# CN-UPB/DeepCoMP

Hardware: AMD Instinct MI355X
Metric: env steps/sec (higher is better)
Workload: dtype f64 positions / f32 rates

## Files before the change

deepcomp_amd/csrc/dcomp_device.h:

```cpp
#pragma once
#include <hip/hip_runtime.h>
#include <stdint.h>

#include "../../include/dcomp_types.h"

#define DCOMP_BLOCK 256
#define DCOMP_WIDE_MIN_B 20
#define DCOMP_SPARSE_MIN_B 7

#define VM_ARRIVED1(a) asm volatile("" : "+v"(a))
#define VM_ARRIVED2(a, b) asm volatile("" : "+v"(a), "+v"(b))
#define VM_ARRIVED3(a, b, c) asm volatile("" : "+v"(a), "+v"(b), "+v"(c))

namespace dcomp {

constexpr float BW = 9e6f;
constexpr float LOG2E = 1.4426950408889634f;
constexpr float TEN_LOG10_2 = 3.0102999566398120f;
constexpr float EPS = 1e-16f;
constexpr float MIN_UTIL = -20.f, MAX_UTIL = 20.f;

struct UeCfg {
    int16_t init_x, init_y;
    uint8_t vel_lo, vel_hi;
// ... 45 lines not shown
    uint32_t maxcap_mask;
    double pl_c1, pl_c2;
    uint32_t time;
    int32_t num_steps;
    int32_t out_every_step;
    int32_t horizon;
    int32_t tight_g;
    int32_t tight_gpw;
    int32_t tight_magic;
    uint32_t episode_inc;
    uint32_t any_sum_mode;
    uint32_t seed_lo, seed_hi, episode;
    uint32_t env_base;
    float half_gamma;
    float log2k;
    float log2k_s;
    double dt2;
    float dt2f;
    uint32_t dsq_exact;
    double bs_x[DCOMP_MASK32_MAX_BS], bs_y[DCOMP_MASK32_MAX_BS];
    int32_t bs_mode[DCOMP_MASK32_MAX_BS];
};

template <int CTRL>
__device__ __forceinline__ float dpp_f32(float v)
{
    return __int_as_float(__builtin_amdgcn_update_dpp(0, __float_as_int(v), CTRL, 0xF, 0xF, true));
}
__device__ __forceinline__ float swz_xor16(float v)
{
    return __int_as_float(__builtin_amdgcn_ds_swizzle(__float_as_int(v), 0x401F));
}
#define DCOMP_DPP_QUAD_X1 0xB1
#define DCOMP_DPP_QUAD_X2 0x4E
#define DCOMP_DPP_HALF_MIRROR 0x141
#define DCOMP_DPP_ROW_MIRROR 0x140

struct OpSum { __device__ __forceinline__ static float f(float a, float b) { return a + b; } };
struct OpMin { __device__ __forceinline__ static float f(float a, float b) { return __builtin_amdgcn_fmed3f(a, b, -3.0e38f); } };
struct OpMax { __device__ __forceinline__ static float f(float a, float b) { return __builtin_amdgcn_fmed3f(a, b, 3.0e38f); } };

template <int W, class Op>
__device__ __forceinline__ float group_reduce(float v)
{
    if (W >= 2) v = Op::f(v, dpp_f32<DCOMP_DPP_QUAD_X1>(v));
    if (W >= 4) v = Op::f(v, dpp_f32<DCOMP_DPP_QUAD_X2>(v));
// ... 107 lines not shown
    return xx + yy;
}
__device__ __noinline__ bool in_range_exact(double px, double py, double bx, double by, double dt2)
{
    return dist_sq_ref(bx - px, by - py) < dt2;
}
__device__ __forceinline__ void pair_eval_q(double px, double py, double bx, double by, const KParams &p, bool &in_range, float &l2snr, float &q);
__device__ __forceinline__ void pair_eval(double px, double py, double bx, double by, const KParams &p, bool &in_range,
                                          float &l2snr, bool &tiny)
{
    float q;
    pair_eval_q(px, py, bx, by, p, in_range, l2snr, q);
    tiny = q < NEAR_D2;
    if (q == p.dt2f || p.dsq_exact) in_range = in_range_exact(px, py, bx, by, p.dt2);
}
__device__ __forceinline__ void pair_eval_q(double px, double py, double bx, double by, const KParams &p, bool &in_range, float &l2snr, float &q)
{
    double dx = bx - px, dy = by - py;
    double dsq = __builtin_fma(dy, dy, dx * dx);
    in_range = dsq < p.dt2;
    q = (float)dsq;
    l2snr = __builtin_fmaf(-p.half_gamma, fast_log2(q * 0x1p-12f), p.log2k_s);
}
__device__ __forceinline__ float pair_eval_tiny(double px, double py, double bx, double by, const KParams &p)
{
    double dx = bx - px, dy = by - py;
    float q = (float)__builtin_fma(dy, dy, dx * dx);
    float d = __builtin_amdgcn_sqrtf(q) + EPS;
    return __builtin_fmaf(-2.0f * p.half_gamma, fast_log2(d), p.log2k);
}
template <int B>
__device__ __forceinline__ uint32_t eval_pairs(double px, double py, const KParams &p, float (&l2)[B], bool *near_wave = nullptr,
                                               const double *bsx = nullptr, const double *bsy = nullptr)
{
    uint32_t in_range = 0;
    float qmin = 3.0e38f;
    const bool vec_form = bsx != nullptr;
    bool edge = false;
    float emin = 3.0e38f;
#pragma unroll
    for (int b = 0; b < B; b++) {
        bool ir;
        float q;
        pair_eval_q(px, py, bsx ? bsx[b] : p.bs_x[b], bsy ? bsy[b] : p.bs_y[b], p, ir, l2[b], q);
        in_range |= (uint32_t)ir << b;
        qmin = min_med3(qmin, q);
        if (vec_form) emin = min_med3(emin, __builtin_fabsf(q - p.dt2f));
        else edge |= q == p.dt2f;
    }
    if (vec_form) edge = emin == 0.f;
    if (__ballot(edge) != 0ull || p.dsq_exact) {
        in_range = 0;
#pragma unroll
        for (int b = 0; b < B; b++)
            in_range |= (uint32_t)in_range_exact(px, py, bsx ? bsx[b] : p.bs_x[b], bsy ? bsy[b] : p.bs_y[b], p.dt2) << b;
    }
    const bool nw = __ballot(qmin < NEAR_D2) != 0ull;
    if (near_wave) *near_wave = nw;
    if (nw) {
#pragma unroll
        for (int b = 0; b < B; b++) {
            const double bx = bsx ? bsx[b] : p.bs_x[b], by = bsy ? bsy[b] : p.bs_y[b];
            float t = pair_eval_tiny(px, py, bx, by, p);
            double dx = bx - px, dy = by - py;
            if ((float)__builtin_fma(dy, dy, dx * dx) < 1e-20f) l2[b] = t;
        }
    }
    return in_range;
}
constexpr float RATE_SMALL_L2 = -6.0f + L2_OFF;
__device__ __forceinline__ float rate_unshared_small(float l2snr, bool &needfix)
{
    needfix = l2snr > RATE_SMALL_L2;
    const float z = fast_exp2(min_med3(l2snr, RATE_SMALL_L2));
    constexpr float K = BW * LOG2E, S1 = 0x1p-24f, S2 = 0x1p-48f, S3 = 0x1p-72f, S4 = 0x1p-96f;
    float t = __builtin_fmaf(z, -0.25f * K * S4, 0.33333334f * K * S3);
    t = __builtin_fmaf(z, t, -0.5f * K * S2);
    t = __builtin_fmaf(z, t, K * S1);
    return z * t;
}
__device__ __forceinline__ float rate_unshared_any(float l2snr)
{
    const float l = l2snr - L2_OFF;
    const float s = fast_exp2(fminf(l, 100.f));
    const float u = 1.0f + s;
    const float lg = fast_log2(u) * (s * fast_rcp(u - 1.0f));
// ... 8 lines not shown
}

__device__ __forceinline__ void philox4x32_10(uint32_t c0, uint32_t c1, uint32_t c2, uint32_t c3, uint32_t k0, uint32_t k1,
                                              uint32_t (&out)[4])
{
#pragma unroll
    for (int r = 0; r < 10; r++) {
        const unsigned long long p0 = (unsigned long long)0xD2511F53u * c0, p1 = (unsigned long long)0xCD9E8D57u * c2;
        const uint32_t hi0 = (uint32_t)(p0 >> 32), lo0 = (uint32_t)p0, hi1 = (uint32_t)(p1 >> 32), lo1 = (uint32_t)p1;
        c0 = hi1 ^ c1 ^ k0; c1 = lo1; c2 = hi0 ^ c3 ^ k1; c3 = lo0;
        k0 += 0x9E3779B9u; k1 += 0xBB67AE85u;
    }
    out[0] = c0; out[1] = c1; out[2] = c2; out[3] = c3;
}

__device__ __forceinline__ unsigned long long mv_pack(uint32_t wx, uint32_t wy, uint32_t vel, uint32_t pausing, uint32_t cp,
                                                      uint32_t cursor)
{
    return (unsigned long long)(wx & 0xFFFF) | ((unsigned long long)(wy & 0xFFFF) << 16) | ((unsigned long long)(vel & 0xFF) << 32) |
           ((unsigned long long)((pausing << 7) | (cp & 0x7Fu)) << 40) | ((unsigned long long)(cursor & 0xFFFF) << 48);
}

constexpr uint32_t UID_BORN = 0x8000u;
__device__ __forceinline__ void draw_triple(const KParams &p, int env, uint32_t uidw, uint32_t k, uint32_t episode, uint32_t &vel,
                                            uint32_t &wx, uint32_t &wy, int mcfg)
{
    const uint32_t id0 = (uidw & 0x7FFFu) - 1u;
    const bool born = (uidw & UID_BORN) != 0u;
    if (p.rng_mode == DCOMP_RNG_TAPE) {
        if (k >= (uint32_t)p.tape_depth) { atomicOr(p.flags, DCOMP_FLAG_TAPE_EMPTY); k = p.tape_depth - 1; }
        const uint32_t slot = born ? (uint32_t)p.U0 + id0 : id0;
        ushort4 t = p.tape_triples[((size_t)env * p.tape_ids + slot) * p.tape_depth + k];
        vel = t.x; wx = t.y; wy = t.z;
        VM_ARRIVED3(vel, wx, wy);
    } else {
        uint32_t r[4] = {0x12345678u + k * 977u, 0x9abcdef0u ^ uidw * 2654435761u, 0x0fedcba9u + (uint32_t)env * 40503u, 0u};
        philox4x32_10(p.env_base + (uint32_t)env, id0 | (born ? UID_BORN : 0u), episode, k + 1, p.seed_lo, p.seed_hi, r);
        const uint32_t vlo = (uint32_t)mcfg & 0xFFu, vhi = ((uint32_t)mcfg >> 8) & 0xFFu, bb = ((uint32_t)mcfg >> 23) & 0xFFu;
        vel = vlo + __umulhi(r[0], vhi - vlo + 1u);
        wx = bb + __umulhi(r[1], (uint32_t)(p.map_w - 2 * (int)bb + 1));
        wy = bb + __umulhi(r[2], (uint32_t)(p.map_h - 2 * (int)bb + 1));
    }
}
template <bool SCALAR>
__device__ __forceinline__ void draw_triple_wave(const KParams &p, int env, uint32_t uidw, uint32_t k, uint32_t episode, bool redraw,
                                                 uint32_t &vel, uint32_t &wx, uint32_t &wy, int mcfg)
{
    if (!SCALAR || p.rng_mode == DCOMP_RNG_TAPE) {
        if (redraw) draw_triple(p, env, uidw, k, episode, vel, wx, wy, mcfg);
        return;
    }
    const int lane = (int)(threadIdx.x & 63u);
    unsigned long long need = __ballot(redraw);
    while (need != 0ull) {
        const int l = __ffsll((long long)need) - 1;
        need &= need - 1ull;
        uint32_t k0 = p.seed_lo, k1 = p.seed_hi, eb = p.env_base;
        asm volatile("" : "+s"(k0), "+s"(k1), "+s"(eb));
        const uint32_t e_s = (uint32_t)__builtin_amdgcn_readlane(env, l), u_s = (uint32_t)__builtin_amdgcn_readlane((int)uidw, l);
        const uint32_t k_s = (uint32_t)__builtin_amdgcn_readlane((int)k, l), m_s = (uint32_t)__builtin_amdgcn_readlane(mcfg, l);
        uint32_t r[4] = {0x12345678u + k_s * 977u, 0x9abcdef0u ^ u_s * 2654435761u, 0x0fedcba9u + e_s * 40503u, 0u};
        philox4x32_10(eb + e_s, ((u_s & 0x7FFFu) - 1u) | (u_s & UID_BORN), episode, k_s + 1u, k0, k1, r);
        const uint32_t vlo = m_s & 0xFFu, vhi = (m_s >> 8) & 0xFFu, bb = (m_s >> 23) & 0xFFu;
        const uint32_t v_s = vlo + __umulhi(r[0], vhi - vlo + 1u);
        const uint32_t x_s = bb + __umulhi(r[1], (uint32_t)(p.map_w - 2 * (int)bb + 1));
        const uint32_t y_s = bb + __umulhi(r[2], (uint32_t)(p.map_h - 2 * (int)bb + 1));
        const bool mine = lane == l;
        vel = mine ? v_s : vel; wx = mine ? x_s : wx; wy = mine ? y_s : wy;
    }
}
__device__ __forceinline__ int load_mv_cfg(const KParams &p, uint32_t uidw)
{
// ... 67 lines not shown
        }
    }
}

template <bool LAT = false>
__device__ __forceinline__ void move_ue(const KParams &p, int env, uint32_t uidw, uint32_t episode, double &px, double &py,
                                        unsigned long long &mv, int mcfg)
{
#pragma clang fp contract(off)
    uint32_t wxi = (uint32_t)(mv & 0xFFFF), wyi = (uint32_t)((mv >> 16) & 0xFFFF), vel = (uint32_t)((mv >> 32) & 0xFF);
    uint32_t pz = (uint32_t)((mv >> 40) & 0xFF), cursor = (uint32_t)(mv >> 48);
    uint32_t pausing = (pz >> 7) & 1, cp = pz & 0x7Fu;
    const uint32_t pause_dur = ((uint32_t)mcfg >> 16) & 0x7Fu;
    double wx = (double)wxi, wy = (double)wyi;
    if (px == wx && py == wy) pausing = 1;
    const bool stay = pausing && cp < pause_dur;
    const bool redraw = pausing && !stay;
    cp = stay ? cp + 1u : cp;
    draw_triple_wave<LAT>(p, env, uidw, cursor, episode, redraw, vel, wxi, wyi, mcfg);
    cursor = redraw ? cursor + 1u : cursor;
    pausing = redraw ? 0u : pausing;
    cp = redraw ? 0u : cp;
    wx = (double)wxi; wy = (double)wyi;
    if (p.ue_velq != nullptr) advance_ue<LAT, true>(p, uidw, vel, stay, wx, wy, px, py);
    else advance_ue<LAT, false>(p, uidw, vel, stay, wx, wy, px, py);
    mv = mv_pack(wxi, wyi, vel, pausing, cp, cursor);
}

enum { MP_GENERIC = 0, MP_RES_FAIR = 1, MP_MIXED = 2 };
template <int MP>
__device__ __forceinline__ int bs_mode_of(const KParams &p, int b)
{
    if (MP == MP_RES_FAIR) return DCOMP_RES_FAIR;
    if (MP == MP_MIXED) return (b % 3 == 0) ? DCOMP_RES_FAIR : (b % 3 == 1) ? DCOMP_RATE_FAIR : DCOMP_PROP_FAIR;
    return p.bs_mode[b];
}

template <int B, int UPAD>
struct Geo {
    static constexpr int WG = UPAD < 64 ? UPAD : 64;
    static constexpr int NW = UPAD > 64 ? UPAD / 64 : 1;
    static constexpr int GPB = DCOMP_BLOCK >= UPAD ? DCOMP_BLOCK / UPAD : 1;
    static constexpr int ROW_MULTI = 4 * B + 1;
};

template <int B>
struct StageGeo {
// ... 42 lines not shown
        v[i] = a;
    }
    __syncthreads();
}

__device__ __noinline__ unsigned long long maxcap_rate_key(double pl_c1, double pl_c2, double px, double py, double bx, double by)
{
#pragma clang fp contract(off)
    const double dx = bx - px, dy = by - py;
    const double d = __builtin_sqrt(dx * dx + dy * dy);
    const double pl = pl_c1 + pl_c2 * log10(d + 1e-16);
    const double snr = pow(10.0, (30.0 - pl) / 10.0) / 1e-9;
    return (unsigned long long)__double_as_longlong(1.0 + snr);
}

template <int B, int UPAD, int MP, class S = SegPadded, bool PRE = false, int CARRY = 0>
__device__ __forceinline__ void shared_rates(const KParams &p, BlockSharedT<B, UPAD> &sh, uint32_t conn, const float (&l2)[B], float ewma,
                                             double px, double py, int u, int idx, int env_local, int wave, int lane, int gbase,
                                             float (&dr)[B], float (&cnt)[B], int near_hint = -1, const S &sg = S{}, const float *prow = nullptr,
                                             float *dru_io = nullptr)
{
    using G = Geo<B, UPAD>;
    float agg[B];
    const float inv_ewma = fast_rcp(ewma + EPS);
    bool fix = false;
#pragma unroll
    for (int b = 0; b < B; b++) {
        const bool c = (conn >> b) & 1u;
        unsigned long long m = __ballot(c);
        float dru = 0.f;
        if (PRE) dru = c ? prow[b] : 0.f;
        else if (CARRY == 2) dru = c ? dru_io[b] : 0.f;
        else if (CARRY == 1) {
            bool f;
            const float t = rate_unshared_small(l2[b], f);
            dru_io[b] = t;
            dru = c ? t : 0.f;
        } else if (m != 0ull) {
            bool f;
            const float t = rate_unshared_small(l2[b], f);
            dru = c ? t : 0.f;
            if (near_hint < 0) fix |= c && f;
        }
        dr[b] = dru;
        cnt[b] = (float)seg_popcount<G::WG>(m, gbase, sg);
    }
    if (!PRE && CARRY != 2 && (near_hint < 0 ? (__ballot(fix) != 0ull) : (near_hint != 0))) {
#pragma unroll
        for (int b = 0; b < B; b++) {
            if (CARRY == 1) { if (l2[b] > RATE_SMALL_L2) { dru_io[b] = rate_unshared_any(l2[b]); if ((conn >> b) & 1u) dr[b] = dru_io[b]; } }
            else if (((conn >> b) & 1u) && l2[b] > RATE_SMALL_L2) dr[b] = rate_unshared_any(l2[b]);
        }
    }
#pragma unroll
    for (int b = 0; b < B; b++) {
        const bool c = (conn >> b) & 1u;
        const int mode = bs_mode_of<MP>(p, b);
        float a = 0.f;
        if (mode == DCOMP_RATE_FAIR) a = c ? fast_rcp(dr[b]) : 0.f;
        else if (mode == DCOMP_PROP_FAIR) a = dr[b] * inv_ewma;
        agg[b] = a;
    }
    if (MP == MP_MIXED) {
        constexpr int NS = B - (B + 2) / 3;
        if (NS > 0) {
            float sv[NS > 0 ? NS : 1];
#pragma unroll
            for (int b = 0, k = 0; b < B; b++) if (b % 3 != 0) sv[k++] = agg[b];
// ... 38 lines not shown
#pragma unroll
        for (int b = 0; b < B; b++) {
            key[b] = 1ull;
            if (heavy && ((contested >> b) & 1u)) key[b] = maxcap_rate_key(p.pl_c1, p.pl_c2, px, py, p.bs_x[b], p.bs_y[b]);
            if ((cand >> b) & 1u) atomicMax(&sh.mc_u[env_local * B + b], key[b]);
        }
        __syncthreads();
#pragma unroll
        for (int b = 0; b < B; b++)
            if (((cand >> b) & 1u) && key[b] == sh.mc_u[env_local * B + b])
                atomicMin(&sh.mc_win[env_local * B + b], ((uint32_t)p.conn_since[(size_t)idx * B + b] << 8) | (uint32_t)u);
        __syncthreads();
#pragma unroll
        for (int b = 0; b < B; b++)
            if (((cand >> b) & 1u) && (sh.mc_win[env_local * B + b] & 0xFFu) == (uint32_t)u) mc_winner |= 1u << b;
        __syncthreads();
    }
#pragma unroll
    for (int b = 0; b < B; b++) {
#pragma clang fp contract(off)
        const bool c = (conn >> b) & 1u;
        const int mode = bs_mode_of<MP>(p, b);
        float dru = dr[b], out = 0.f;
        if (mode == DCOMP_RES_FAIR) out = dru * fast_rcp(fmaxf(cnt[b], 1.f));
        else if (mode == DCOMP_RATE_FAIR) out = fast_rcp(agg[b]);
        else if (mode == DCOMP_PROP_FAIR) out = (dru * inv_ewma) * fast_rcp(agg[b] + EPS) * dru;
        else out = ((mc_winner >> b) & 1u) ? dru : 0.f;
        dr[b] = (mode == DCOMP_RES_FAIR || mode == DCOMP_PROP_FAIR) ? out : (c ? out : 0.f);
    }
}

struct Outs { float *obs, *reward, *sum_util, *ue_dr, *ue_util, *rb_out; uint8_t *next_act; int compact; };

template <int B, class F>
__device__ __forceinline__ int policy_action_fn(const KParams &p, uint32_t conn, F dr)
{
    float mx = dr(0);
    int best = 0;
#pragma unroll 4
    for (int b = 1; b < B; b++) { const float d = dr(b); if (d > mx) { mx = d; best = b; } }
    if (p.policy == DCOMP_POLICY_3GPP) return ((conn >> best) & 1u) ? 0 : conn ? __builtin_ffs((int)conn) : best + 1;
    uint32_t sel = B == 32 ? ~0u : (1u << (B & 31)) - 1u;
    if (p.policy == DCOMP_POLICY_DYNAMIC) {
        const float thr = mx * p.policy_eps;
        sel = 0;
#pragma unroll 4
        for (int b = 0; b < B; b++) sel |= (dr(b) >= thr ? 1u : 0u) << b;
    } else if (p.policy == DCOMP_POLICY_CLUSTER) { sel = p.policy_cluster[best]; VM_ARRIVED1(sel); }
    const uint32_t drop = conn & ~sel;
    if (drop) return __builtin_ffs((int)drop);
    const uint32_t cand = sel & ~conn;
    float m2 = -__builtin_huge_valf();
    int a = 0;
#pragma unroll 4
    for (int b = 0; b < B; b++) { const float d = dr(b); if (((cand >> b) & 1u) && d > m2) { m2 = d; a = b + 1; } }
// ... 5 lines not shown
{
    float mx = dr[0];
    int best = 0;
#pragma unroll
    for (int b = 1; b < B; b++) if (dr[b] > mx) { mx = dr[b]; best = b; }
    if (p.policy == DCOMP_POLICY_3GPP)
        return ((conn >> best) & 1u) ? 0 : conn ? __builtin_ffs((int)conn) : best + 1;
    uint32_t sel = B == 32 ? ~0u : (1u << (B & 31)) - 1u;
    if (p.policy == DCOMP_POLICY_DYNAMIC) {
        const float thr = mx * p.policy_eps;
        sel = 0;
#pragma unroll
        for (int b = 0; b < B; b++) sel |= (dr[b] >= thr ? 1u : 0u) << b;
    } else if (p.policy == DCOMP_POLICY_CLUSTER) { sel = p.policy_cluster[best]; VM_ARRIVED1(sel); }
    const uint32_t drop = conn & ~sel;
    if (drop) return __builtin_ffs((int)drop);
    const uint32_t cand = sel & ~conn;
    float m2 = -__builtin_huge_valf();
    int a = 0;
#pragma unroll
    for (int b = 0; b < B; b++) if (((cand >> b) & 1u) && dr[b] > m2) { m2 = dr[b]; a = b + 1; }
    return a;
}
template <int B, int UPAD, bool RESET, bool DYN = false, bool STAGED = true, class S = SegPadded, int POL = -1, int KIND = -1>
__device__ __forceinline__ void write_outputs(const KParams &p, const Outs &o, BlockSharedT<B, UPAD> &sh, bool active, int env, int env_local, int u, int idx,
                                              int wave, int lane, int gbase, uint32_t conn, uint32_t in_range,
                                              float (&l2)[B], float (&cnt)[B], float util, float curr_dr,
                                              float reward_before, bool alive, int n_eff, const S &sg = S{}, uint32_t *pol_next = nullptr)
{
    using G = Geo<B, UPAD>;
    using SG = StageGeo<B>;
    const int U = p.U;
    const int kind = KIND >= 0 ? KIND : p.kind;
    float tsum[B];
#pragma unroll
    for (int b = 0; b < B; b++) tsum[b] = ((conn >> b) & 1u) ? util : 0.f;
    if (!RESET && kind == DCOMP_MULTI) {
        seg_reduce_vec<G::WG, OpSum, B>(tsum, sg, lane);
        if (G::NW > 1) xwave_reduce_<B, G::NW, OpSum>(tsum, sh, wave, lane);
    }
    float l2max = l2[0];
#pragma unroll
    for (int b = 1; b < B; b++) l2max = fmaxf(l2max, l2[b]);

    float reward = 0.f;
    if (kind == DCOMP_CENTRAL) {
        float r[1];
        if (p.reward_agg == DCOMP_REWARD_MIN) {
            r[0] = seg_reduce<G::WG, OpMin>(alive ? reward_before : 1.f, sg, lane);
            xwave_reduce_<1, G::NW, OpMin>(r, sh, wave, lane);
        } else {
            r[0] = seg_reduce<G::WG, OpSum>(alive ? reward_before : 0.f, sg, lane);
            xwave_reduce_<1, G::NW, OpSum>(r, sh, wave, lane);
            if (p.reward_agg == DCOMP_REWARD_AVG) r[0] = r[0] * fast_rcp((float)n_eff);
        }
        reward = r[0];
    } else if (!RESET) {
        reward = util;
        if (p.reward_agg == DCOMP_REWARD_SUM) {
            sh.nb_conn[threadIdx.x] = alive ? conn : 0u;
            sh.nb_rb[threadIdx.x] = reward_before;
            __syncthreads();
            if (in_range != 0) {
                float s = 0.f;
                const int base = (int)threadIdx.x - u;
                for (int v = 0; v < U; v++) if (sh.nb_conn[base + v] & conn) s += sh.nb_rb[base + v];
                reward = s;
            }
            __syncthreads();
        } else {
            if (p.reward_agg == DCOMP_REWARD_AVG) {
                float n = 0.f, t = 0.f;
#pragma unroll
                for (int b = 0; b < B; b++) {
                    const float ind = (float)((in_range >> b) & 1u);
                    n = __builtin_fmaf(ind, cnt[b], n);
                    t = __builtin_fmaf(ind, tsum[b], t);
                }
                if (n > 0.f) {
                    const bool lone = conn == 0u;
                    reward = (lone ? t + util : t) * fast_rcp(lone ? n + 1.f : n);
                }
            } else {
                float tmin[B];
#pragma unroll
                for (int b = 0; b < B; b++) tmin[b] = ((conn >> b) & 1u) ? util : MAX_UTIL;
                seg_reduce_vec<G::WG, OpMin, B>(tmin, sg, lane);
                if (G::NW > 1) xwave_reduce_<B, G::NW, OpMin>(tmin, sh, wave, lane);
                float m = util;
#pragma unroll
                for (int b = 0; b < B; b++) if ((in_range >> b) & 1u) m = fminf(m, cnt[b] > 0.f ? tmin[b] : MAX_UTIL);
                reward = (in_range != 0) ? m : util;
            }
        }
    }

    if (o.sum_util) {
        float s[1];
        s[0] = seg_reduce<G::WG, OpSum>(alive ? util : 0.f, sg, lane);
        xwave_reduce_<1, G::NW, OpSum>(s, sh, wave, lane);
        if (active && u == 0) o.sum_util[env] = s[0];
    }
    if (active) {
        if (o.ue_dr) stream_store(&o.ue_dr[idx], alive ? curr_dr : 0.f);
        if (o.ue_util) stream_store(&o.ue_util[idx], alive ? util : 0.f);
        if (o.rb_out) stream_store(&o.rb_out[idx], alive ? reward_before : 0.f);
    }

    const float inv_u = fast_rcp((float)n_eff);
    const bool live = DYN ? alive : true;
    const float util_n = live ? util * (1.0f / MAX_UTIL) : 0.f;
    float env_cols[DYN ? 2 * B : 1];
#pragma unroll
    for (int b = 0; b < B; b++) {
        l2[b] = live ? fast_exp2(l2[b] - l2max) : 0.f;
        const float avg = tsum[b] * fast_rcp(fmaxf(cnt[b], 1.f)) * (1.0f / MAX_UTIL);
        if (DYN) { env_cols[b] = cnt[b] * inv_u; env_cols[B + b] = avg; }
        tsum[b] = live ? avg : 0.f;
        cnt[b] = live ? cnt[b] * inv_u : 0.f;
    }
    if (POL != 0 && (POL == 1 || o.next_act)) {
        const int a = policy_action<B>(p, conn, l2);
        if (active && o.next_act) o.next_act[idx] = (uint8_t)(live ? a : 0);
        if (pol_next) *pol_next = live ? (uint32_t)a : 0u;
    }
    if (kind == DCOMP_MULTI && !STAGED) {
        if (active && o.compact) {
            if (o.reward) o.reward[idx] = alive ? reward : 0.f;
            float *rec = o.obs + (size_t)idx * (B + 2) + (size_t)env * (2 * B);
            float recv[B + 2];
#pragma unroll
            for (int b = 0; b < B; b++) recv[b] = l2[b];
            recv[B] = util_n;
            recv[B + 1] = __uint_as_float(conn);
            store_run<B + 2>(rec, recv);
            if (u == U - 1) {
                float tl[2 * B];
#pragma unroll
                for (int b = 0; b < B; b++) { tl[b] = cnt[b]; tl[B + b] = tsum[b]; }
                store_run<2 * B>(rec + B + 2, tl);
            }
        } else if (active) {
            if (o.reward) o.reward[idx] = alive ? reward : 0.f;
            float rowv[SG::ROW];
#pragma unroll
            for (int b = 0; b < B; b++) {
                rowv[b] = (float)((conn >> b) & 1u);
                rowv[B + b] = l2[b];
                rowv[2 * B + b] = cnt[b];
                rowv[3 * B + b] = tsum[b];
            }
            rowv[4 * B] = util_n;
            store_run<SG::ROW>(o.obs + (size_t)idx * SG::ROW, rowv);
        }
    } else if (kind == DCOMP_MULTI && o.compact) {
        if (active && o.reward) stream_store(&o.reward[idx], alive ? reward : 0.f);
        const unsigned long long am = __ballot(active);
        if (am != 0ull) {
            constexpr int CW = B + 2;
            const int first = __ffsll((long long)am) - 1, last = 63 - __clzll((long long)am);
            const int idx0 = __builtin_amdgcn_readlane(idx, first), env0 = __builtin_amdgcn_readlane(env, first);
            const size_t g0 = (size_t)idx0 * CW + (size_t)env0 * (2 * B);
            const int loc = (idx - idx0) * CW + (env - env0) * (2 * B);
            const bool tail = u == U - 1;
            const int n = __builtin_amdgcn_readlane(loc + CW + (tail ? 2 * B : 0), last);
            const int ph = (int)((((size_t)o.obs >> 2) + g0) & 3);
            uint32_t *st = reinterpret_cast<uint32_t *>(sh.stage[wave]);
            constexpr int CH = (SG::WORDS - 4) & ~3;
            const bool one = n <= CH;
#pragma unroll 1
            for (int w0 = 0; w0 < n; w0 += CH) {
                const int cw = min(CH, n - w0);
                if (active) {
                    uint32_t *rec = st + ph - w0 + loc;
                    const int at = loc - w0;
#pragma unroll
                    for (int b = 0; b < B; b++) if (one || (unsigned)(at + b) < (unsigned)cw) rec[b] = __float_as_uint(l2[b]);
                    if (one || (unsigned)(at + B) < (unsigned)cw) rec[B] = __float_as_uint(util_n);
                    if (one || (unsigned)(at + B + 1) < (unsigned)cw) rec[B + 1] = conn;
                    if (tail) {
#pragma unroll
                        for (int b = 0; b < B; b++) {
                            if (one || (unsigned)(at + CW + b) < (unsigned)cw) rec[CW + b] = __float_as_uint(DYN ? env_cols[b] : cnt[b]);
                            if (one || (unsigned)(at + CW + B + b) < (unsigned)cw) rec[CW + B + b] = __float_as_uint(DYN ? env_cols[B + b] : tsum[b]);
                        }
                    }
                }
                wave_lds_fence();
                const int n_end = ph + cw;
                uint32_t *gbase_ptr = reinterpret_cast<uint32_t *>(o.obs) + g0 + w0 - ph;
                for (int j = lane * 4; j < n_end; j += 256) {
                    if (j >= ph && j + 4 <= n_end) {
                        typedef uint32_t u4v __attribute__((ext_vector_type(4)));
                        __builtin_nontemporal_store(*reinterpret_cast<const u4v *>(st + j), reinterpret_cast<u4v *>(gbase_ptr + j));
                    } else {
                        for (int k = max(j, ph); k < min(j + 4, n_end); k++) gbase_ptr[k] = st[k];
                    }
                }
                wave_lds_fence();
            }
        }
    } else if (kind == DCOMP_MULTI) {
        if (active && o.reward) stream_store(&o.reward[idx], alive ? reward : 0.f);
        const unsigned long long am = __ballot(active);
        const int nrows = group_popcount<64>(am, 0);
        const int row0 = __builtin_amdgcn_readlane(idx, am ? __ffsll((long long)am) - 1 : 0);
        const int r = idx - row0;
        float *st = sh.stage[wave];
#pragma unroll 1
        for (int pass = 0; pass < SG::NPASS; pass++) {
            const int rbase = pass * SG::RPP;
            if (rbase >= nrows) break;
            const int rows = min(SG::RPP, nrows - rbase);
            const size_t g0 = (size_t)(row0 + rbase) * SG::ROW;
            const int ph = (int)((((size_t)o.obs >> 2) + g0) & 3);
            if (active && r >= rbase && r < rbase + rows) {
                float *row = st + ph + (r - rbase) * SG::ROW;
#pragma unroll
                for (int b = 0; b < B; b++) {
                    row[b] = (float)((conn >> b) & 1u);
                    row[B + b] = l2[b];
                    row[2 * B + b] = cnt[b];
                    row[3 * B + b] = tsum[b];
                }
                row[4 * B] = util_n;
            }
            wave_lds_fence();
            const int n_end = ph + rows * SG::ROW;
            float *gbase_ptr = o.obs + g0 - ph;
            for (int j = lane * 4; j < n_end; j += 256) {
                if (j >= ph && j + 4 <= n_end) {
                    typedef float f4v __attribute__((ext_vector_type(4)));
                    __builtin_nontemporal_store(*reinterpret_cast<const f4v *>(st + j), reinterpret_cast<f4v *>(gbase_ptr + j));
                } else {
                    for (int k = max(j, ph); k < min(j + 4, n_end); k++) gbase_ptr[k] = st[k];
                }
            }
            wave_lds_fence();
        }
    } else if (G::NW == 1 && STAGED) {
        if (active && o.reward && u == 0) o.reward[env] = reward;
        const unsigned long long am = __ballot(active);
        if (am != 0ull) {
            const int REC = U * (2 * B + 1);
            const int env0 = __builtin_amdgcn_readlane(env, __ffsll((long long)am) - 1);
            const int envl = __builtin_amdgcn_readlane(env, 63 - __clzll((long long)am));
            const int n = (envl - env0 + 1) * REC;
            const size_t g0 = (size_t)env0 * REC;
            const int ph = (int)((((size_t)o.obs >> 2) + g0) & 3);
            float *st = sh.stage[wave];
            constexpr int CH = (SG::WORDS - 4) & ~3;
            const int o_conn = (env - env0) * REC + u * B, o_dr = o_conn + U * B, o_ut = (env - env0) * REC + 2 * U * B + u;
#pragma unroll 1
            for (int w0 = 0; w0 < n; w0 += CH) {
                const int cnt = min(CH, n - w0);
                if (active) {
                    float *row = st + ph - w0;
                    const bool one = n <= CH;
#pragma unroll
                    for (int b = 0; b < B; b++) {
                        if (one || (unsigned)(o_conn + b - w0) < (unsigned)cnt) row[o_conn + b] = (float)((conn >> b) & 1u);
                        if (one || (unsigned)(o_dr + b - w0) < (unsigned)cnt) row[o_dr + b] = l2[b];
                    }
                    if (one || (unsigned)(o_ut - w0) < (unsigned)cnt) row[o_ut] = util_n;
                }
                wave_lds_fence();
                const int n_end = ph + cnt;
                float *gbase_ptr = o.obs + g0 + w0 - ph;
                for (int j = lane * 4; j < n_end; j += 256) {
                    if (j >= ph && j + 4 <= n_end) {
                        typedef float f4v __attribute__((ext_vector_type(4)));
                        __builtin_nontemporal_store(*reinterpret_cast<const f4v *>(st + j), reinterpret_cast<f4v *>(gbase_ptr + j));
                    } else {
                        for (int k = max(j, ph); k < min(j + 4, n_end); k++) gbase_ptr[k] = st[k];
                    }
                }
                wave_lds_fence();
            }
        }
    } else if (active) {
        if (o.reward && u == 0) o.reward[env] = reward;
        float *base = o.obs + (size_t)env * U * (2 * B + 1);
        float cv[B];
#pragma unroll
        for (int b = 0; b < B; b++) cv[b] = (float)((conn >> b) & 1u);
        store_run<B>(base + u * B, cv);
        store_run<B>(base + U * B + u * B, l2);
        base[2 * U * B + u] = util_n;
    }
}

__device__ __forceinline__ void reset_ue(const KParams &p, int env, int u, uint32_t episode, double &px, double &py, unsigned long long &mv)
{
    const UeCfg c = p.ue_cfg[u];
    int x, y;
    if (p.rng_mode == DCOMP_RNG_TAPE) { const size_t t = (size_t)env * p.U0 + u; x = p.tape_pos0[2 * t]; y = p.tape_pos0[2 * t + 1]; }
    else {
        uint32_t r[4];
        philox4x32_10(p.env_base + (uint32_t)env, (uint32_t)u, episode, 0u, p.seed_lo, p.seed_hi, r);
        x = (int)__umulhi(r[0], (uint32_t)p.map_w + 1u);
        y = (int)__umulhi(r[1], (uint32_t)p.map_h + 1u);
    }
    if (c.init_x >= 0) x = c.init_x;
    if (c.init_y >= 0) y = c.init_y;
    px = (double)x; py = (double)y;
    uint32_t vel, wx, wy;
    draw_triple(p, env, (uint32_t)u + 1u, 0u, episode, vel, wx, wy, mv_cfg_pack(c.vel_lo, c.vel_hi, c.pause, c.border));
    mv = mv_pack(wx, wy, vel, 0u, 0u, 1u);
}

__device__ __forceinline__ void store_state(const KParams &p, int idx, double px, double py, unsigned long long mv, uint32_t conn, float ewma)
{
    p.pos[idx] = make_double2(px, py);
    p.mv[idx] = mv;
    p.conn[idx] = conn;
    p.ewma[idx] = ewma;
}

template <int B>
struct PairCarry { float l2[B]; float dru[B]; uint32_t in_range; bool near; };

template <int B, int UPAD, int MP, bool STORE, class S, int POL = -1, bool CARRY = false, int KIND = -1>
__device__ __forceinline__ void step_once(const KParams &p, BlockSharedT<B, UPAD> &sh, const Outs &o, bool emit, bool active, int env,
                                          int env_local, int u, int idx, int wave, int lane, int gbase, uint32_t act, uint32_t time,
                                          uint32_t episode, bool step_util, float dr_req, int vrange, double &px, double &py,
                                          unsigned long long &mv, uint32_t &conn, float &ewma, const S &sg, uint32_t *pol_next = nullptr,
                                          const double *bsx = nullptr, const double *bsy = nullptr, PairCarry<B> *carry = nullptr,
                                          int env_shift = 0, int idx_shift = 0)
{
    float l2[B], dr[B], cnt[B];
    uint32_t in_range = B >= 32 ? 0xFFFFFFFFu : ((1u << (B & 31)) - 1u);
    bool near_pre = false, near_post = false;
    if (act > (uint32_t)B) { atomicOr(p.flags, DCOMP_FLAG_BAD_ACTION); act = 0; }
    constexpr bool SPARSE_OK = STORE && B >= DCOMP_SPARSE_MIN_B && 64 * (B + 1) <= StageGeo<B>::WORDS;
    if (SPARSE_OK && !(MP == MP_GENERIC && p.any_maxcap)) {
        float *const prow = sh.stage[wave] + lane * (B + 1);
        const uint32_t act_bit = act ? 1u << (act - 1u) : 0u;
        uint32_t need = active ? (conn | act_bit) : 0u, inr_old = 0u;
        while (__ballot(need != 0u) != 0ull) {
            if (need != 0u) {
                const int b = __ffs((int)need) - 1;
                need &= need - 1u;
                const double2 bp = sh.bs[b];
                bool ir, near;
                float l;
                pair_eval(px, py, bp.x, bp.y, p, ir, l, near);
// ... 37 lines not shown
        if ((unsigned long long)__double_as_longlong(px) > (unsigned long long)__double_as_longlong((double)p.map_w) ||
            (unsigned long long)__double_as_longlong(py) > (unsigned long long)__double_as_longlong((double)p.map_h)) atomicOr(p.flags, DCOMP_FLAG_OUTSIDE_MAP);
    }
    in_range = eval_pairs<B>(px, py, p, l2, &near_post, bsx, bsy);
    if (CARRY) {
#pragma unroll
        for (int b = 0; b < B; b++) carry->l2[b] = l2[b];
        carry->in_range = in_range; carry->near = near_post;
    }
    conn &= in_range;
    float stale = 0.f;
#pragma unroll
    for (int b = 0; b < B; b++)
        stale += __int_as_float(__float_as_int(dr[b]) & __builtin_amdgcn_sbfe((int)conn, b, 1));
    ewma = __builtin_fmaf(0.9f, stale, 0.1f * ewma);
    if (CARRY) shared_rates<B, UPAD, MP, S, false, 1>(p, sh, conn, l2, ewma, px, py, u, idx, env_local, wave, lane, gbase, dr, cnt, (int)near_post, sg, nullptr, carry->dru);
    else shared_rates<B, UPAD, MP, S>(p, sh, conn, l2, ewma, px, py, u, idx, env_local, wave, lane, gbase, dr, cnt, (int)near_post, sg);
    curr = 0.f;
#pragma unroll
    for (int b = 0; b < B; b++) curr += dr[b];
    const float util = ue_utility(curr, step_util, dr_req);
    if (STORE && active) store_state(p, idx, px, py, mv, conn, ewma);
    if (emit) {
        Outs o2 = o;
        if (POL != 0 && o2.next_act) o2.next_act -= idx_shift;
        write_outputs<B, UPAD, false, false, STORE, S, POL, KIND>(p, o2, sh, active, env + env_shift, env_local, u, idx + idx_shift, wave, lane, gbase, conn,
                                                         in_range, l2, cnt, util, curr, reward_before, active, p.U, sg, pol_next);
    }
}

__device__ __forceinline__ double in_vgpr(double v)
{
    asm volatile("" : "+v"(v));
    return v;
}

__device__ __forceinline__ int xcd_contiguous_block()
{
    const unsigned b = blockIdx.x, n = gridDim.x, q = n >> 3, r = n & 7u, x = b & 7u;
    return (int)(x * q + (x < r ? x : r) + (b >> 3));
}

template <int B, int UPAD, int MP, bool ROLLOUT, bool TIGHT = false, int POL = -1, int KIND = -1>
__device__ __forceinline__ void step_kernel_body(const KParams &p, BlockSharedT<B, UPAD> &sh)
{
    using G = Geo<B, UPAD>;
    const int tid = threadIdx.x, lane = tid & 63, wave = tid >> 6;
    int env_local = tid / UPAD, u = tid % UPAD;
    const int blk = ROLLOUT ? (int)blockIdx.x : xcd_contiguous_block();
    int env = blk * G::GPB + env_local;
    bool active = (env < p.E) && (u < p.U);
    int gbase = lane & ~(G::WG - 1);
    using S = SegT<TIGHT>;
    S sg{};
    if constexpr (TIGHT) {
        const int g = p.tight_g, gi = (lane * p.tight_magic) >> 16;
        u = lane - gi * g;
// ... 9 lines not shown
        if (tid < B) sh.bs[tid] = make_double2(p.bs_x[tid], p.bs_y[tid]);
        __syncthreads();
    }
    double px = 0.0, py = 0.0;
    unsigned long long mv = 0;
    uint32_t conn = 0, act = 0;
    float ewma = 0.f;
    bool step_util = false;
    float dr_req = 1.f;
    int vrange = MV_CFG_ARRIVED;
    if (active) {
        double2 q = p.pos[idx];
        px = q.x; py = q.y;
        mv = p.mv[idx];
        conn = p.conn[idx];
        ewma = p.ewma[idx];
        if (!ROLLOUT) act = p.action[idx];
        {
            const UeCfg c = p.ue_cfg[u];
            step_util = c.util == DCOMP_UTIL_STEP; dr_req = c.dr_req;
            vrange = mv_cfg_pack(c.vel_lo, c.vel_hi, c.pause, c.border);
        }
    }
    Outs o{p.obs, p.reward, p.sum_util, p.ue_dr, p.ue_util, p.rb_out, POL == 0 ? nullptr : p.next_act, p.obs_compact};
    if (!ROLLOUT) {
        step_once<B, UPAD, MP, true, S, -1, false, KIND>(p, sh, o, true, active, env, env_local, u, idx, wave, lane, gbase, act, p.time, p.episode,
                                                         step_util, dr_req, vrange, px, py, mv, conn, ewma, sg);
    } else {
        const int T = p.num_steps;
        const size_t EU = (size_t)p.E * p.U;
        uint32_t time = p.time, episode = p.episode;
        double bsx[B], bsy[B];
#pragma unroll
        for (int b = 0; b < B; b++) { bsx[b] = in_vgpr(p.bs_x[b]); bsy[b] = in_vgpr(p.bs_y[b]); }
        PairCarry<B> carry;
        auto refresh_carry = [&]() {
            carry.in_range = eval_pairs<B>(px, py, p, carry.l2, &carry.near, bsx, bsy);
#pragma unroll
            for (int b = 0; b < B; b++) {
                bool f;
                carry.dru[b] = rate_unshared_small(carry.l2[b], f);
                if (f) carry.dru[b] = rate_unshared_any(carry.l2[b]);
            }
        };
        refresh_carry();
        const uint8_t *actp = p.action + (active ? idx : 0);
        const bool ploop = POL != 0 && p.policy_loop;
        const int TT = ploop ? 1 : T;
        uint32_t pol_next = 0u;
        uint32_t nb[8];
        auto load_chunk = [&](int t0) {
#pragma unroll
            for (int j = 0; j < 8; j++) nb[j] = (uint32_t)actp[(size_t)min(t0 + j, TT - 1) * EU];
        };
        load_chunk(0);
        unsigned long long act_cur = 0ull;
        int env_shift = 0, idx_shift = 0;
#pragma unroll 1
        for (int t = 0; t < T; t++) {
            if (p.horizon > 0 && time == (uint32_t)p.horizon) {
                episode += p.episode_inc;
                time = 0;
                conn = 0u; ewma = 0.f;
                if (active) reset_ue(p, env, u, episode, px, py, mv);
                refresh_carry();
            }
            if ((t & 7) == 0) {
                const uint32_t lo = nb[0] | (nb[1] << 8) | (nb[2] << 16) | (nb[3] << 24), hi = nb[4] | (nb[5] << 8) | (nb[6] << 16) | (nb[7] << 24);
                act_cur = ((unsigned long long)hi << 32) | lo;
                load_chunk(t + 8);
            }
            act = active ? (uint32_t)(act_cur >> (8 * (t & 7))) & 0xFFu : 0u;
            if (ploop && t > 0) act = active ? pol_next : 0u;
            step_once<B, UPAD, MP, false, S, POL, true, KIND>(p, sh, o, p.out_every_step || t == T - 1 || ploop, active, env, env_local, u, idx, wave, lane,
                                                        gbase, act, time, episode, step_util, dr_req, vrange, px, py, mv, conn, ewma, sg,
                                                        POL != 0 ? &pol_next : nullptr, bsx, bsy, &carry, env_shift, idx_shift);
            time += 1;
            if (p.out_every_step) { env_shift += p.E; idx_shift += (int)EU; }
            if ((MP == MP_GENERIC && p.any_maxcap) || ((KIND >= 0 ? KIND : p.kind) == DCOMP_MULTI && p.reward_agg == DCOMP_REWARD_SUM)) __syncthreads();
        }
    }
    if (ROLLOUT && active) store_state(p, idx, px, py, mv, conn, ewma);
}

template <int B, int UPAD, int MP>
__global__ __launch_bounds__(DCOMP_BLOCK) void step_kernel(const KParams p)
{
    __shared__ BlockSharedT<B, UPAD> sh;
    step_kernel_body<B, UPAD, MP, false>(p, sh);
}

template <int B, int UPAD, int MP, int KIND = -1>
__global__ __launch_bounds__(DCOMP_BLOCK) void step_kernel_tight(const KParams p)
{
    __shared__ BlockSharedT<B, UPAD> sh;
    step_kernel_body<B, UPAD, MP, false, true, -1, KIND>(p, sh);
}

template <int B, int UPAD, int MP, int POL, int KIND = -1>
__global__ __launch_bounds__(DCOMP_BLOCK) void rollout_kernel(const KParams p)
{
    __shared__ BlockSharedT<B, UPAD> sh;
    step_kernel_body<B, UPAD, MP, true, false, POL, KIND>(p, sh);
}

// ... 127 lines not shown
```

Measured before the change: 852.2 million.

## Rematerialize kernel args in SGPRs and use output presence bitmask in rollout loop

Adds asm-barrier helpers that pin loop-invariant kernel parameters and output pointers in scalar registers, or re-read them from the kernarg segment at the point of use, so they are not held live across the rollout loop. Output pointer null checks become a single scalar bitmask, and the resource-fair path uses an integer count when there is one wave per group. The goal is lower register pressure and fewer spills or VGPR copies in the hot rollout loop, at the cost of extra scalar loads and inline asm constraints that can block compiler optimizations.

```diff
diff --git a/deepcomp_amd/csrc/dcomp_device.h b/deepcomp_amd/csrc/dcomp_device.h
--- a/deepcomp_amd/csrc/dcomp_device.h
+++ b/deepcomp_amd/csrc/dcomp_device.h
@@ -91,6 +91,20 @@
     int32_t bs_mode[DCOMP_MASK32_MAX_BS];
 };
 
+template <bool ON, class T>
+__device__ __forceinline__ T tested_here(T v)
+{
+    if (ON) asm volatile("" : "+s"(v));
+    return v;
+}
+
+__device__ __forceinline__ const KParams &args_reread()
+{
+    auto a = __builtin_amdgcn_kernarg_segment_ptr();
+    asm volatile("" : "+s"(a));
+    return *(const KParams *)a;
+}
+
 template <int CTRL>
 __device__ __forceinline__ float dpp_f32(float v)
 {
@@ -244,12 +258,13 @@
     q = (float)dsq;
     l2snr = __builtin_fmaf(-p.half_gamma, fast_log2(q * 0x1p-12f), p.log2k_s);
 }
+template <bool LOOP = false>
 __device__ __forceinline__ float pair_eval_tiny(double px, double py, double bx, double by, const KParams &p)
 {
     double dx = bx - px, dy = by - py;
     float q = (float)__builtin_fma(dy, dy, dx * dx);
     float d = __builtin_amdgcn_sqrtf(q) + EPS;
-    return __builtin_fmaf(-2.0f * p.half_gamma, fast_log2(d), p.log2k);
+    return __builtin_fmaf(-2.0f * p.half_gamma, fast_log2(d), tested_here<LOOP>(p.log2k));
 }
 template <int B>
 __device__ __forceinline__ uint32_t eval_pairs(double px, double py, const KParams &p, float (&l2)[B], bool *near_wave = nullptr,
@@ -271,7 +286,7 @@
         else edge |= q == p.dt2f;
     }
     if (vec_form) edge = emin == 0.f;
-    if (__ballot(edge) != 0ull || p.dsq_exact) {
+    if (__ballot(edge) != 0ull || (vec_form ? tested_here<true>(p.dsq_exact) : p.dsq_exact)) {
         in_range = 0;
 #pragma unroll
         for (int b = 0; b < B; b++)
@@ -283,7 +298,7 @@
 #pragma unroll
         for (int b = 0; b < B; b++) {
             const double bx = bsx ? bsx[b] : p.bs_x[b], by = bsy ? bsy[b] : p.bs_y[b];
-            float t = pair_eval_tiny(px, py, bx, by, p);
+            float t = vec_form ? pair_eval_tiny<true>(px, py, bx, by, p) : pair_eval_tiny(px, py, bx, by, p);
             double dx = bx - px, dy = by - py;
             if ((float)__builtin_fma(dy, dy, dx * dx) < 1e-20f) l2[b] = t;
         }
@@ -338,13 +353,14 @@
 }
 
 constexpr uint32_t UID_BORN = 0x8000u;
+template <bool LOOP = false>
 __device__ __forceinline__ void draw_triple(const KParams &p, int env, uint32_t uidw, uint32_t k, uint32_t episode, uint32_t &vel,
                                             uint32_t &wx, uint32_t &wy, int mcfg)
 {
     const uint32_t id0 = (uidw & 0x7FFFu) - 1u;
     const bool born = (uidw & UID_BORN) != 0u;
     if (p.rng_mode == DCOMP_RNG_TAPE) {
-        if (k >= (uint32_t)p.tape_depth) { atomicOr(p.flags, DCOMP_FLAG_TAPE_EMPTY); k = p.tape_depth - 1; }
+        if (k >= (uint32_t)p.tape_depth) { atomicOr(p.flags, DCOMP_FLAG_TAPE_EMPTY); k = tested_here<LOOP>(p.tape_depth) - 1; }
         const uint32_t slot = born ? (uint32_t)p.U0 + id0 : id0;
         ushort4 t = p.tape_triples[((size_t)env * p.tape_ids + slot) * p.tape_depth + k];
         vel = t.x; wx = t.y; wy = t.z;
@@ -363,7 +379,7 @@
                                                  uint32_t &vel, uint32_t &wx, uint32_t &wy, int mcfg)
 {
     if (!SCALAR || p.rng_mode == DCOMP_RNG_TAPE) {
-        if (redraw) draw_triple(p, env, uidw, k, episode, vel, wx, wy, mcfg);
+        if (redraw) draw_triple<SCALAR>(p, env, uidw, k, episode, vel, wx, wy, mcfg);
         return;
     }
     const int lane = (int)(threadIdx.x & 63u);
@@ -477,7 +493,7 @@
     pausing = redraw ? 0u : pausing;
     cp = redraw ? 0u : cp;
     wx = (double)wxi; wy = (double)wyi;
-    if (p.ue_velq != nullptr) advance_ue<LAT, true>(p, uidw, vel, stay, wx, wy, px, py);
+    if (tested_here<LAT>(p.ue_velq) != nullptr) advance_ue<LAT, true>(p, uidw, vel, stay, wx, wy, px, py);
     else advance_ue<LAT, false>(p, uidw, vel, stay, wx, wy, px, py);
     mv = mv_pack(wxi, wyi, vel, pausing, cp, cursor);
 }
@@ -566,6 +582,7 @@
 {
     using G = Geo<B, UPAD>;
     float agg[B];
+    int cnt_i[B];
     const float inv_ewma = fast_rcp(ewma + EPS);
     bool fix = false;
 #pragma unroll
@@ -587,7 +604,8 @@
             if (near_hint < 0) fix |= c && f;
         }
         dr[b] = dru;
-        cnt[b] = (float)seg_popcount<G::WG>(m, gbase, sg);
+        cnt_i[b] = seg_popcount<G::WG>(m, gbase, sg);
+        cnt[b] = (float)cnt_i[b];
     }
     if (!PRE && CARRY != 2 && (near_hint < 0 ? (__ballot(fix) != 0ull) : (near_hint != 0))) {
 #pragma unroll
@@ -672,7 +690,8 @@
         const bool c = (conn >> b) & 1u;
         const int mode = bs_mode_of<MP>(p, b);
         float dru = dr[b], out = 0.f;
-        if (mode == DCOMP_RES_FAIR) out = dru * fast_rcp(fmaxf(cnt[b], 1.f));
+        if (MP == MP_RES_FAIR && G::NW == 1) out = dru * fast_rcp((float)max(cnt_i[b], 1));
+        else if (mode == DCOMP_RES_FAIR) out = dru * fast_rcp(fmaxf(cnt[b], 1.f));
         else if (mode == DCOMP_RATE_FAIR) out = fast_rcp(agg[b]);
         else if (mode == DCOMP_PROP_FAIR) out = (dru * inv_ewma) * fast_rcp(agg[b] + EPS) * dru;
         else out = ((mc_winner >> b) & 1u) ? dru : 0.f;
@@ -680,7 +699,34 @@
     }
 }
 
-struct Outs { float *obs, *reward, *sum_util, *ue_dr, *ue_util, *rb_out; uint8_t *next_act; int compact; };
+enum { OUT_REWARD = 1, OUT_SUM_UTIL = 2, OUT_UE_DR = 4, OUT_UE_UTIL = 8, OUT_RB = 16, OUT_NEXT_ACT = 32 };
+template <class T>
+__device__ __forceinline__ T *in_sgpr(T *v)
+{
+    auto g = (__attribute__((address_space(1))) T *)v;
+    asm volatile("" : "+s"(g));
+    return (T *)g;
+}
+template <bool MASK, bool REREAD = false>
+struct OutsT {
+    float *obs, *reward, *sum_util, *ue_dr, *ue_util, *rb_out; uint8_t *next_act; int compact;
+    uint32_t have_bits;
+    __device__ __forceinline__ OutsT at_emit() const
+    {
+        if (!REREAD) return *this;
+        const KParams &a = args_reread();
+        return OutsT{in_sgpr(a.obs), in_sgpr(a.reward), in_sgpr(a.sum_util), in_sgpr(a.ue_dr), in_sgpr(a.ue_util), in_sgpr(a.rb_out),
+                     next_act ? a.next_act : nullptr, compact, have_bits};
+    }
+    __device__ __forceinline__ bool have(uint32_t bit, const void *ptr) const
+    {
+        if (!MASK) return ptr != nullptr;
+        uint32_t h = have_bits;
+        asm volatile("" : "+s"(h));
+        return (h & bit) != 0u;
+    }
+};
+using Outs = OutsT<false>;
 
 template <int B, class F>
 __device__ __forceinline__ int policy_action_fn(const KParams &p, uint32_t conn, F dr)
@@ -732,16 +778,19 @@
     for (int b = 0; b < B; b++) if (((cand >> b) & 1u) && dr[b] > m2) { m2 = dr[b]; a = b + 1; }
     return a;
 }
-template <int B, int UPAD, bool RESET, bool DYN = false, bool STAGED = true, class S = SegPadded, int POL = -1, int KIND = -1>
-__device__ __forceinline__ void write_outputs(const KParams &p, const Outs &o, BlockSharedT<B, UPAD> &sh, bool active, int env, int env_local, int u, int idx,
+template <int B, int UPAD, bool RESET, bool DYN = false, bool STAGED = true, class S = SegPadded, int POL = -1, int KIND = -1, class O = Outs>
+__device__ __forceinline__ void write_outputs(const KParams &p, const O &o, BlockSharedT<B, UPAD> &sh, bool active, int env, int env_local, int u, int idx,
                                               int wave, int lane, int gbase, uint32_t conn, uint32_t in_range,
                                               float (&l2)[B], float (&cnt)[B], float util, float curr_dr,
                                               float reward_before, bool alive, int n_eff, const S &sg = S{}, uint32_t *pol_next = nullptr)
 {
     using G = Geo<B, UPAD>;
     using SG = StageGeo<B>;
-    const int U = p.U;
+    const int U = tested_here<!STAGED>(p.U);
     const int kind = KIND >= 0 ? KIND : p.kind;
+    const auto reward_agg = [&]() { return tested_here<!STAGED>(p.reward_agg); };
+    int u_first = u;
+    if (!STAGED) asm volatile("" : "+v"(u_first));
     float tsum[B];
 #pragma unroll
     for (int b = 0; b < B; b++) tsum[b] = ((conn >> b) & 1u) ? util : 0.f;
@@ -756,18 +805,18 @@
     float reward = 0.f;
     if (kind == DCOMP_CENTRAL) {
         float r[1];
-        if (p.reward_agg == DCOMP_REWARD_MIN) {
+        if (reward_agg() == DCOMP_REWARD_MIN) {
             r[0] = seg_reduce<G::WG, OpMin>(alive ? reward_before : 1.f, sg, lane);
             xwave_reduce_<1, G::NW, OpMin>(r, sh, wave, lane);
         } else {
             r[0] = seg_reduce<G::WG, OpSum>(alive ? reward_before : 0.f, sg, lane);
             xwave_reduce_<1, G::NW, OpSum>(r, sh, wave, lane);
-            if (p.reward_agg == DCOMP_REWARD_AVG) r[0] = r[0] * fast_rcp((float)n_eff);
+            if (reward_agg() == DCOMP_REWARD_AVG) r[0] = r[0] * fast_rcp((float)n_eff);
         }
         reward = r[0];
     } else if (!RESET) {
         reward = util;
-        if (p.reward_agg == DCOMP_REWARD_SUM) {
+        if (reward_agg() == DCOMP_REWARD_SUM) {
             sh.nb_conn[threadIdx.x] = alive ? conn : 0u;
             sh.nb_rb[threadIdx.x] = reward_before;
             __syncthreads();
@@ -779,7 +828,7 @@
             }
             __syncthreads();
         } else {
-            if (p.reward_agg == DCOMP_REWARD_AVG) {
+            if (reward_agg() == DCOMP_REWARD_AVG) {
                 float n = 0.f, t = 0.f;
 #pragma unroll
                 for (int b = 0; b < B; b++) {
@@ -805,16 +854,16 @@
         }
     }
 
-    if (o.sum_util) {
+    if (o.have(OUT_SUM_UTIL, o.sum_util)) {
         float s[1];
         s[0] = seg_reduce<G::WG, OpSum>(alive ? util : 0.f, sg, lane);
         xwave_reduce_<1, G::NW, OpSum>(s, sh, wave, lane);
-        if (active && u == 0) o.sum_util[env] = s[0];
+        if (active && u_first == 0) o.sum_util[env] = s[0];
     }
     if (active) {
-        if (o.ue_dr) stream_store(&o.ue_dr[idx], alive ? curr_dr : 0.f);
-        if (o.ue_util) stream_store(&o.ue_util[idx], alive ? util : 0.f);
-        if (o.rb_out) stream_store(&o.rb_out[idx], alive ? reward_before : 0.f);
+        if (o.have(OUT_UE_DR, o.ue_dr)) stream_store(&o.ue_dr[idx], alive ? curr_dr : 0.f);
+        if (o.have(OUT_UE_UTIL, o.ue_util)) stream_store(&o.ue_util[idx], alive ? util : 0.f);
+        if (o.have(OUT_RB, o.rb_out)) stream_store(&o.rb_out[idx], alive ? reward_before : 0.f);
     }
 
     const float inv_u = fast_rcp((float)n_eff);
@@ -829,14 +878,14 @@
         tsum[b] = live ? avg : 0.f;
         cnt[b] = live ? cnt[b] * inv_u : 0.f;
     }
-    if (POL != 0 && (POL == 1 || o.next_act)) {
+    if (POL != 0 && (POL == 1 || o.have(OUT_NEXT_ACT, o.next_act))) {
         const int a = policy_action<B>(p, conn, l2);
-        if (active && o.next_act) o.next_act[idx] = (uint8_t)(live ? a : 0);
+        if (active && o.have(OUT_NEXT_ACT, o.next_act)) o.next_act[idx] = (uint8_t)(live ? a : 0);
         if (pol_next) *pol_next = live ? (uint32_t)a : 0u;
     }
     if (kind == DCOMP_MULTI && !STAGED) {
         if (active && o.compact) {
-            if (o.reward) o.reward[idx] = alive ? reward : 0.f;
+            if (o.have(OUT_REWARD, o.reward)) o.reward[idx] = alive ? reward : 0.f;
             float *rec = o.obs + (size_t)idx * (B + 2) + (size_t)env * (2 * B);
             float recv[B + 2];
 #pragma unroll
@@ -851,7 +900,7 @@
                 store_run<2 * B>(rec + B + 2, tl);
             }
         } else if (active) {
-            if (o.reward) o.reward[idx] = alive ? reward : 0.f;
+            if (o.have(OUT_REWARD, o.reward)) o.reward[idx] = alive ? reward : 0.f;
             float rowv[SG::ROW];
 #pragma unroll
             for (int b = 0; b < B; b++) {
@@ -864,7 +913,7 @@
             store_run<SG::ROW>(o.obs + (size_t)idx * SG::ROW, rowv);
         }
     } else if (kind == DCOMP_MULTI && o.compact) {
-        if (active && o.reward) stream_store(&o.reward[idx], alive ? reward : 0.f);
+        if (active && o.have(OUT_REWARD, o.reward)) stream_store(&o.reward[idx], alive ? reward : 0.f);
         const unsigned long long am = __ballot(active);
         if (am != 0ull) {
             constexpr int CW = B + 2;
@@ -911,7 +960,7 @@
             }
         }
     } else if (kind == DCOMP_MULTI) {
-        if (active && o.reward) stream_store(&o.reward[idx], alive ? reward : 0.f);
+        if (active && o.have(OUT_REWARD, o.reward)) stream_store(&o.reward[idx], alive ? reward : 0.f);
         const unsigned long long am = __ballot(active);
         const int nrows = group_popcount<64>(am, 0);
         const int row0 = __builtin_amdgcn_readlane(idx, am ? __ffsll((long long)am) - 1 : 0);
@@ -949,7 +998,7 @@
             wave_lds_fence();
         }
     } else if (G::NW == 1 && STAGED) {
-        if (active && o.reward && u == 0) o.reward[env] = reward;
+        if (active && o.have(OUT_REWARD, o.reward) && u == 0) o.reward[env] = reward;
         const unsigned long long am = __ballot(active);
         if (am != 0ull) {
             const int REC = U * (2 * B + 1);
@@ -989,7 +1038,7 @@
             }
         }
     } else if (active) {
-        if (o.reward && u == 0) o.reward[env] = reward;
+        if (o.have(OUT_REWARD, o.reward) && u_first == 0) o.reward[env] = reward;
         float *base = o.obs + (size_t)env * U * (2 * B + 1);
         float cv[B];
 #pragma unroll
@@ -1030,8 +1079,8 @@
 template <int B>
 struct PairCarry { float l2[B]; float dru[B]; uint32_t in_range; bool near; };
 
-template <int B, int UPAD, int MP, bool STORE, class S, int POL = -1, bool CARRY = false, int KIND = -1>
-__device__ __forceinline__ void step_once(const KParams &p, BlockSharedT<B, UPAD> &sh, const Outs &o, bool emit, bool active, int env,
+template <int B, int UPAD, int MP, bool STORE, class S, int POL = -1, bool CARRY = false, int KIND = -1, class O = Outs>
+__device__ __forceinline__ void step_once(const KParams &p, BlockSharedT<B, UPAD> &sh, const O &o, bool emit, bool active, int env,
                                           int env_local, int u, int idx, int wave, int lane, int gbase, uint32_t act, uint32_t time,
                                           uint32_t episode, bool step_util, float dr_req, int vrange, double &px, double &py,
                                           unsigned long long &mv, uint32_t &conn, float &ewma, const S &sg, uint32_t *pol_next = nullptr,
@@ -1115,9 +1164,9 @@
     const float util = ue_utility(curr, step_util, dr_req);
     if (STORE && active) store_state(p, idx, px, py, mv, conn, ewma);
     if (emit) {
-        Outs o2 = o;
-        if (POL != 0 && o2.next_act) o2.next_act -= idx_shift;
-        write_outputs<B, UPAD, false, false, STORE, S, POL, KIND>(p, o2, sh, active, env + env_shift, env_local, u, idx + idx_shift, wave, lane, gbase, conn,
+        O o2 = o.at_emit();
+        if (POL != 0 && o2.have(OUT_NEXT_ACT, o2.next_act)) o2.next_act -= idx_shift;
+        write_outputs<B, UPAD, false, false, STORE, S, POL, KIND, O>(p, o2, sh, active, env + env_shift, env_local, u, idx + idx_shift, wave, lane, gbase, conn,
                                                          in_range, l2, cnt, util, curr, reward_before, active, p.U, sg, pol_next);
     }
 }
@@ -1126,6 +1175,13 @@
 {
     asm volatile("" : "+v"(v));
     return v;
+}
+template <class T>
+__device__ __forceinline__ T *in_vgpr(T *v)
+{
+    auto g = (__attribute__((address_space(1))) T *)v;
+    asm volatile("" : "+v"(g));
+    return (T *)g;
 }
 
 __device__ __forceinline__ int xcd_contiguous_block()
@@ -1181,11 +1237,18 @@
             vrange = mv_cfg_pack(c.vel_lo, c.vel_hi, c.pause, c.border);
         }
     }
-    Outs o{p.obs, p.reward, p.sum_util, p.ue_dr, p.ue_util, p.rb_out, POL == 0 ? nullptr : p.next_act, p.obs_compact};
     if (!ROLLOUT) {
+        const Outs o{p.obs, p.reward, p.sum_util, p.ue_dr, p.ue_util, p.rb_out, POL == 0 ? nullptr : p.next_act, p.obs_compact};
         step_once<B, UPAD, MP, true, S, -1, false, KIND>(p, sh, o, true, active, env, env_local, u, idx, wave, lane, gbase, act, p.time, p.episode,
                                                          step_util, dr_req, vrange, px, py, mv, conn, ewma, sg);
     } else {
+        using O = OutsT<true, TIGHT>;
+        uint8_t *const next_act = POL == 0 ? nullptr : p.next_act;
+        const uint32_t have = (p.reward ? OUT_REWARD : 0u) | (p.sum_util ? OUT_SUM_UTIL : 0u) | (p.ue_dr ? OUT_UE_DR : 0u) | (p.ue_util ? OUT_UE_UTIL : 0u) |
+                              (p.rb_out ? OUT_RB : 0u) | (next_act ? OUT_NEXT_ACT : 0u);
+        const O o = TIGHT ? O{nullptr, nullptr, nullptr, nullptr, nullptr, nullptr, next_act, p.obs_compact, have}
+                          : O{in_vgpr(p.obs), in_vgpr(p.reward), in_vgpr(p.sum_util), in_vgpr(p.ue_dr), in_vgpr(p.ue_util), in_vgpr(p.rb_out),
+                              POL == 0 ? nullptr : in_vgpr(next_act), p.obs_compact, have};
         const int T = p.num_steps;
         const size_t EU = (size_t)p.E * p.U;
         uint32_t time = p.time, episode = p.episode;
@@ -1217,11 +1280,14 @@
         int env_shift = 0, idx_shift = 0;
 #pragma unroll 1
         for (int t = 0; t < T; t++) {
-            if (p.horizon > 0 && time == (uint32_t)p.horizon) {
+            const int horizon = tested_here<true>(p.horizon), every = tested_here<true>(p.out_every_step);
+            S sg_t = sg;
+            if constexpr (TIGHT) sg_t.g = tested_here<true>(sg.g);
+            if (horizon > 0 && time == (uint32_t)horizon) {
                 episode += p.episode_inc;
                 time = 0;
                 conn = 0u; ewma = 0.f;
-                if (active) reset_ue(p, env, u, episode, px, py, mv);
+                if (active) reset_ue(args_reread(), env, u, episode, px, py, mv);
                 refresh_carry();
             }
             if ((t & 7) == 0) {
@@ -1231,15 +1297,15 @@
             }
             act = active ? (uint32_t)(act_cur >> (8 * (t & 7))) & 0xFFu : 0u;
             if (ploop && t > 0) act = active ? pol_next : 0u;
-            step_once<B, UPAD, MP, false, S, POL, true, KIND>(p, sh, o, p.out_every_step || t == T - 1 || ploop, active, env, env_local, u, idx, wave, lane,
-                                                        gbase, act, time, episode, step_util, dr_req, vrange, px, py, mv, conn, ewma, sg,
+            step_once<B, UPAD, MP, false, S, POL, true, KIND, O>(p, sh, o, every || t == T - 1 || ploop, active, env, env_local, u, idx, wave, lane,
+                                                        gbase, act, time, episode, step_util, dr_req, vrange, px, py, mv, conn, ewma, sg_t,
                                                         POL != 0 ? &pol_next : nullptr, bsx, bsy, &carry, env_shift, idx_shift);
             time += 1;
-            if (p.out_every_step) { env_shift += p.E; idx_shift += (int)EU; }
-            if ((MP == MP_GENERIC && p.any_maxcap) || ((KIND >= 0 ? KIND : p.kind) == DCOMP_MULTI && p.reward_agg == DCOMP_REWARD_SUM)) __syncthreads();
-        }
-    }
-    if (ROLLOUT && active) store_state(p, idx, px, py, mv, conn, ewma);
+            if (every) { env_shift += p.E; idx_shift += (int)EU; }
+            if ((MP == MP_GENERIC && p.any_maxcap) || ((KIND >= 0 ? KIND : p.kind) == DCOMP_MULTI && tested_here<true>(p.reward_agg) == DCOMP_REWARD_SUM)) __syncthreads();
+        }
+    }
+    if (ROLLOUT && active) store_state(args_reread(), idx, px, py, mv, conn, ewma);
 }
 
 template <int B, int UPAD, int MP>
```

Result: no change. 850.8 million (median of 3 runs) (-0.2%).
